# XinShuo-ph/gaussian_splatting_with_eye_tracking

Measured on AMD Instinct MI355X. Metric: rendered views/sec (fwd+bwd) at 1080p, 1M Gaussians; achieved HBM GB/s %, higher is better.
Workload: dtype fp32; 1 GPU

## Files before the change

gaussian_splatting_with_eye_tracking_amd/csrc/gs_api.cpp:

```cpp
#include <hip/hip_runtime.h>

#include <atomic>
#include <cstdio>
#include <cstdlib>
#include <chrono>
#include <cstring>
#include <functional>
#include <algorithm>
#include <deque>
#include <mutex>
#include <stdexcept>
#include <string>
#include <unordered_set>
#include <utility>
#include <vector>

#include "../../include/gsplat_amd.h"
#include "gs_kernels.h"
#include "gs_layout.h"

using namespace gsamd;

namespace {

thread_local std::string g_err;


struct GsError : std::runtime_error {
    using std::runtime_error::runtime_error;
};

#define GS_HIP_NOTHROW(expr) (void)(expr)
#define GS_HIP(expr)                                                                                  \
    do {                                                                                              \
        hipError_t _e = (expr);                                                                       \
        if (_e != hipSuccess)                                                                         \
            throw GsError(std::string(#expr) + " failed: " + hipGetErrorString(_e) + " at " __FILE__ \
                          ":" + std::to_string(__LINE__));                                            \
    } while (0)

constexpr int kStages = 15;
const char* kStageNames[kStages] = {"preprocess", "tile_scan",    "duplicate",   "sort_tiles",
                                    "render",     "render_bwd",   "bwd_gauss",   "amr_levels",
                                    "amr_render", "amr_interp",   "knn",         "zero_accum",
                                    "count_tiles", "multiview_bwd", "amr_lists"};
enum Stage {
    kPre, kScan, kDup, kSort, kRender, kRenderBwd, kBwdGauss, kAmrLevels, kAmrRender, kAmrInterp, kKnn, kZero, kCount,
    kMultiView, kAmrLists
};
struct Profiler {
    bool on = false;
    uint32_t mask = ~0u;
    struct Pending { int stage; hipEvent_t a, b; };
    std::vector<Pending> pending;
    double total_ms[kStages] = {0};
    long count[kStages] = {0};
    std::vector<hipEvent_t> pool;
    hipEvent_t get() {
        if (!pool.empty()) { hipEvent_t e = pool.back(); pool.pop_back(); return e; }
        hipEvent_t e; GS_HIP_NOTHROW(hipEventCreate(&e)); return e;
    }
    void harvest() {
        for (auto& p : pending) {
            float ms = 0.f;
            if (hipEventSynchronize(p.b) == hipSuccess && hipEventElapsedTime(&ms, p.a, p.b) == hipSuccess) {
                total_ms[p.stage] += ms; count[p.stage] += 1;
            }
            pool.push_back(p.a); pool.push_back(p.b);
        }
        pending.clear();
    }
};
Profiler g_prof;
std::mutex g_prof_mu;

thread_local DispatchEvents t_dispatch;

struct StageTimer {
    int stage; hipStream_t s; hipEvent_t a = nullptr, b = nullptr; bool on_dispatch;
    StageTimer(int st, hipStream_t str, bool dispatch = false) : stage(st), s(str), on_dispatch(dispatch) {
        if (!g_prof.on || !((g_prof.mask >> st) & 1u)) return;
        std::lock_guard<std::mutex> l(g_prof_mu);
        a = g_prof.get(); b = g_prof.get();
        if (on_dispatch) t_dispatch = DispatchEvents{a, b};
        else hipEventRecord(a, s);
    }
    ~StageTimer() {
        if (!a) return;
        if (on_dispatch) {
            const bool taken = t_dispatch.start == nullptr;
            t_dispatch = DispatchEvents{};
            std::lock_guard<std::mutex> l(g_prof_mu);
            if (taken) {
                g_prof.pending.push_back({stage, a, b});
            } else {
                g_prof.pool.push_back(a);
                g_prof.pool.push_back(b);
            }
            return;
        }
        hipEventRecord(b, s);
        std::lock_guard<std::mutex> l(g_prof_mu);
        g_prof.pending.push_back({stage, a, b});
    }
};

void stage_check(bool debug, hipStream_t s, const char* stage) {
    hipError_t e = hipGetLastError();
    if (e == hipSuccess && debug) e = hipStreamSynchronize(s);
    if (e != hipSuccess) throw GsError(std::string("[HIP ERROR] in stage ") + stage + ": " + hipGetErrorString(e));
}

uint32_t* pinned_words() {
    thread_local uint32_t* p = nullptr;
    if (!p) {
        void* q = nullptr;
        GS_HIP(hipHostMalloc(&q, 64, hipHostMallocDefault));
        p = static_cast<uint32_t*>(q);
    }
    return p;
}

int g_hdr_mirror = -1;

bool hdr_mirror_on() {
    if (g_hdr_mirror < 0) {
        const char* e = std::getenv("GSAMD_HDR_MIRROR");
        g_hdr_mirror = (e && std::atoi(e) == 0) ? 0 : 2;
    }
    return g_hdr_mirror != 0;
}
// ... 203 lines not shown
    in.store_cov3d = t_store_cov3d != 0;
    in.fwd_zero = t_fwd_zero != 0 && grad;
    in.step0_unfilled = amr && t_amr_step0_unfilled != 0;
    if (amr) t_amr_step0_unfilled = 0;
    return in;
}

PreprocessArgs make_pp(const ForwardIn& in, int tile) {
    PreprocessArgs a;
    a.P = in.P;
    a.D = in.D;
    a.M = in.M;
    a.means3D = in.means3D;
    a.scales = in.scales;
    a.scale_modifier = in.scale_modifier;
    a.rotations = in.rotations;
    a.opacities = in.opacities;
    a.shs = in.shs;
    a.cov3D_precomp = in.cov3D_precomp;
    a.colors_precomp = in.colors_precomp;
    a.viewmatrix = in.viewmatrix;
    a.projmatrix = in.projmatrix;
    a.cam_pos = in.cam_pos;
    a.W = in.width;
    a.H = in.height;
    a.tan_fovx = in.tan_fovx;
    a.tan_fovy = in.tan_fovy;
    a.focal_y = (float)in.height / (2.0f * in.tan_fovy);
    a.focal_x = (float)in.width / (2.0f * in.tan_fovx);
    a.block = tile;
    a.prefiltered = in.prefiltered;
    a.store_cov3d = in.store_cov3d;
    a.store_drgb = in.store_drgb;
    a.zero_words = nullptr;
    a.zero_n = 0;
    a.err_token = 0;
    a.antialiasing = in.antialiasing;
    return a;
}

struct Binned {
    GeomView g;
    ImageView img;
    BinningView b;
    AmrBinningView ab;
    int K;
    int T;
    int* radii;
};

int tile_count(int W, int H, int tile) { return ((W + tile - 1) / tile) * ((H + tile - 1) / tile); }

ImageView image_view(char* image, int W, int H, int tile) {
    ImageView v;
    carve_image(image, (size_t)W * H, tile_count(W, H, tile), &v, tile);
    return v;
}

Binned carve_buffers(char* geom, char* binning, char* image, int P, int K, int W, int H, int tile,
                     bool amr = false) {
    Binned r{};
    r.K = K;
    r.T = tile_count(W, H, tile);
    carve_geom(geom, P, &r.g);
    r.img = image_view(image, W, H, tile);
    carve_binning(binning, K, &r.b, amr ? &r.ab : nullptr);
    r.radii = r.g.radii;
    return r;
}

int rendered_count(int hint, char* geom, int P, const char* binning, hipStream_t s, const char* missing) {
    int K = hint;
    if (K < 0) {
        GeomView g;
        carve_geom(geom, P, &g);
        uint32_t hdr[4];
        read_header(g.hdr, hdr, s);
        K = (int)hdr[kHdrNumRendered];
    }
    if (K > 0 && !binning) throw GsError(missing);
    return K;
}

Binned preprocess_and_bin(const ForwardIn& in, const gs_buffer& geometry, const gs_buffer& binning,
                          const gs_buffer& image, int* radii, int tile, bool debug, hipStream_t s,
                          const std::function<void(Binned&)>& before_k = nullptr, int fused_sort_max = 0) {
    Binned r;
    const int W = in.width, H = in.height;
    const int gx = (W + tile - 1) / tile, gy = (H + tile - 1) / tile;
    r.T = gx * gy;
    const size_t N = (size_t)W * H;
    const bool tail = in.store_cov3d || (in.colors_precomp == nullptr && in.store_drgb);
    char* gbase = call_resize(geometry, carve_geom(nullptr, in.P, nullptr, tail, tile == 32), "geometry");
    carve_geom(gbase, in.P, &r.g);
    set_accum_clean(r.g.grad_accum, false);
    char* ibase = call_resize(image, carve_image(nullptr, N, r.T, nullptr, tile), "image");
    carve_image(ibase, N, r.T, &r.img, tile);
    r.radii = radii ? radii : r.g.radii;
    const bool lds_bin = r.T <= kLdsTiles;
    if (r.T == 0) GS_HIP(hipMemsetAsync(r.g.hdr, 0, kHdrWords * sizeof(uint32_t), s));
    if (r.T > 0 && !lds_bin) GS_HIP(hipMemsetAsync(r.img.tile_count, 0, sizeof(uint32_t) * kBinSlots * r.T, s));
    PreprocessArgs pa = make_pp(in, tile);
    pa.err_token = next_error_token();
    set_drgb_written(r.g.drgb, pa.store_drgb && in.colors_precomp == nullptr);
    if (r.T > 0 && lds_bin) {
        pa.zero_words = r.img.tile_count;
        pa.zero_n = kBinSlots * r.T;
    }
    { StageTimer _t(kPre, s); launch_preprocess(pa, r.g, r.radii, lds_bin ? nullptr : r.img.tile_count, s); }
    stage_check(debug, s, "preprocess");
    if (lds_bin) { StageTimer _t(kCount, s); launch_count_tiles(in.P, r.g, r.radii, W, H, tile, r.img, s); }
    stage_check(debug, s, "count_tiles");
    const std::pair<uint32_t*, uint32_t*> mirror =
        (r.T > 0 && hdr_mirror_on()) ? mirror_words() : std::pair<uint32_t*, uint32_t*>{nullptr, nullptr};
    const bool amr = tile == 32;
    bool dup_done = false;
    const SpecKey skey = spec_key(W, H, in.P);
    const size_t cap = (!amr && !before_k && r.T > 0 && !debug) ? spec_capacity(skey) : 0;
    const uint32_t mtoken = mirror.second ? next_mirror_token() : 0u;
    const bool pub_dup = cap > 0 && mirror.second != nullptr;
    if (r.T > 0) { StageTimer _t(kScan, s); launch_tile_scan(r.T, r.img, r.g.hdr, s, pub_dup ? nullptr : mirror.second, bin_slots_for(in.P, gx, gy, tile), gx, dup_banded(gx, gy, tile), pub_dup ? 0u : mtoken); }
    stage_check(debug, s, "tile_scan");
    uint32_t hdr[4];
    if (before_k) {
        begin_header_read(r.g.hdr, s, mirror.first);
        before_k(r);
        finish_header_read(hdr, mirror.first, s, r.g.hdr);
    } else if (cap > 0) {
        begin_header_read(r.g.hdr, s, mirror.first);
        char* sbase = call_resize(binning, carve_binning(nullptr, cap, nullptr), "binning");
        carve_binning(sbase, cap, &r.b);
        { StageTimer _t(kDup, s); launch_duplicate(in.P, r.g, r.radii, W, H, tile, r.img, r.b, s, (uint32_t)cap, r.g.hdr, (uint32_t)cap, pub_dup ? mirror.second : nullptr, pub_dup ? mtoken : 0u); }
        finish_header_read(hdr, mirror.first, s, r.g.hdr);
        dup_done = hdr[kHdrNumRendered] <= cap;
    } else if (mirror.first) {
        begin_header_read(r.g.hdr, s, mirror.first);
        finish_header_read(hdr, mirror.first, s, r.g.hdr);
    } else {
        read_header(r.g.hdr, hdr, s);
    }
    if (in.prefiltered && hdr[kHdrError] == pa.err_token)
        throw GsError("Point is filtered although prefiltered is set. This shouldn't happen!");
    r.K = (int)hdr[kHdrNumRendered];
    if (!amr) note_k(skey, r.K);
    if (!dup_done) {
        char* bbase = call_resize(binning, carve_binning(nullptr, r.K, nullptr, nullptr, amr), "binning");
        carve_binning(bbase, r.K, &r.b, amr ? &r.ab : nullptr);
    }
    if (r.K > 0) {
        if (!dup_done) { StageTimer _t(kDup, s); launch_duplicate(in.P, r.g, r.radii, W, H, tile, r.img, r.b, s, (uint32_t)r.K); }
        stage_check(debug, s, "duplicate");
        { StageTimer _t(kSort, s); launch_sort_tiles(r.T, r.img, r.b, (int)hdr[kHdrMaxTileCount], (int)hdr[kHdrNumLargeTiles], s, fused_sort_max); }
        stage_check(debug, s, "sort_tiles");
    }
    return r;
}

}

DispatchEvents gsamd::take_dispatch_events() {
    const DispatchEvents e = t_dispatch;
    t_dispatch = DispatchEvents{};
    return e;
}

extern "C" {

int gs_abi_version(void) { return GSPLAT_AMD_ABI_VERSION; }

#ifndef GSAMD_DIGEST
#define GSAMD_DIGEST "unstamped"
#endif
const char* gs_build_digest(void) { return GSAMD_DIGEST; }

const char* gs_last_error(void) { return g_err.c_str(); }

namespace {
int base_forward_impl(const ForwardIn& in, const gs_buffer& geometry, const gs_buffer& binning,
                      const gs_buffer& image, float* out_color, int* radii, bool aux, float* out_depth,
                      float* out_alpha, int debug, void* stream, const char* who) {
    const int P = in.P, width = in.width, height = in.height;
    if (aux && (!out_depth || !out_alpha)) throw GsError(std::string(who) + ": out_depth / out_alpha is NULL");
    hipStream_t s = static_cast<hipStream_t>(stream);
    if (P <= 0) {
        if (aux) {
            const size_t N = (width > 0 && height > 0) ? (size_t)width * (size_t)height : 0;
            if (N) {
                GS_HIP(hipMemsetAsync(out_depth, 0, sizeof(float) * N, s));
                GS_HIP(hipMemsetAsync(out_alpha, 0, sizeof(float) * N, s));
            }
        }
        return 0;
    }
    Binned r = preprocess_and_bin(in, geometry, binning, image, radii, 16, debug != 0, s);
    const float* feats = in.colors_precomp ? in.colors_precomp : r.g.rgb;
    bool zeroed;
    {
        StageTimer _t(kRender, s, true);
        const bool zero = in.fwd_zero;
        zeroed = launch_render_forward(width, height, r.img, r.b, r.g, feats, in.background, out_color, s,
                                       zero ? r.g.grad_accum : nullptr, zero ? (size_t)kGradRow * (size_t)P : 0,
                                       reinterpret_cast<uint8_t*>(r.b.scratch));
    }
    if (zeroed) set_accum_clean(r.g.grad_accum, true);
    stage_check(debug != 0, s, "render");
    if (aux) {
        launch_render_forward_aux(width, height, r.img, r.b, r.g, out_depth, out_alpha, s);
        stage_check(debug != 0, s, "render_aux");
    }
    return r.K;
}
}

int gs_rasterizer_forward(gs_buffer geometry, gs_buffer binning, gs_buffer image, int P, int D, int M,
                          const float* background, int width, int height, const float* means3D, const float* shs,
                          const float* colors_precomp, const float* opacities, const float* scales,
                          float scale_modifier, const float* rotations, const float* cov3D_precomp,
                          const float* viewmatrix, const float* projmatrix, const float* cam_pos, float tan_fovx,
                          float tan_fovy, int prefiltered, float* out_color, int* radii, int debug, void* stream) {
    const ForwardIn in = forward_in(false, P, D, M, background, width, height, means3D, shs, colors_precomp, opacities,
                                    scales, scale_modifier, rotations, cov3D_precomp, viewmatrix, projmatrix, cam_pos,
                                    tan_fovx, tan_fovy, prefiltered);
    return guarded([&]() -> int {
        return base_forward_impl(in, geometry, binning, image, out_color, radii, false, nullptr, nullptr, debug,
                                 stream, "gs_rasterizer_forward");
    });
}

int gs_rasterizer_forward_aux(gs_buffer geometry, gs_buffer binning, gs_buffer image, int P, int D, int M,
                              const float* background, int width, int height, const float* means3D, const float* shs,
                              const float* colors_precomp, const float* opacities, const float* scales,
                              float scale_modifier, const float* rotations, const float* cov3D_precomp,
                              const float* viewmatrix, const float* projmatrix, const float* cam_pos, float tan_fovx,
                              float tan_fovy, int prefiltered, float* out_color, int* radii, float* out_depth,
                              float* out_alpha, int debug, void* stream) {
    const ForwardIn in = forward_in(false, P, D, M, background, width, height, means3D, shs, colors_precomp, opacities,
                                    scales, scale_modifier, rotations, cov3D_precomp, viewmatrix, projmatrix, cam_pos,
                                    tan_fovx, tan_fovy, prefiltered);
    return guarded([&]() -> int {
        return base_forward_impl(in, geometry, binning, image, out_color, radii, true, out_depth, out_alpha, debug,
                                 stream, "gs_rasterizer_forward_aux");
    });
}

int gs_rasterizer_forward_ex(gs_buffer geometry, gs_buffer binning, gs_buffer image, int P, int D, int M,
                             const float* background, int width, int height, const float* means3D, const float* shs,
                             const float* colors_precomp, const float* opacities, const float* scales,
                             float scale_modifier, const float* rotations, const float* cov3D_precomp,
                             const float* viewmatrix, const float* projmatrix, const float* cam_pos, float tan_fovx,
                             float tan_fovy, int prefiltered, int antialiasing, float* out_color, int* radii,
                             float* out_depth, float* out_alpha, int debug, void* stream) {
    ForwardIn in = forward_in(false, P, D, M, background, width, height, means3D, shs, colors_precomp, opacities,
                              scales, scale_modifier, rotations, cov3D_precomp, viewmatrix, projmatrix, cam_pos,
                              tan_fovx, tan_fovy, prefiltered);
    in.antialiasing = antialiasing != 0;
    return guarded([&]() -> int {
        if ((out_depth == nullptr) != (out_alpha == nullptr))
            throw GsError("gs_rasterizer_forward_ex: out_depth and out_alpha go together (both, or both NULL)");
        return base_forward_impl(in, geometry, binning, image, out_color, radii, out_depth != nullptr, out_depth,
                                 out_alpha, debug, stream, "gs_rasterizer_forward_ex");
    });
}

namespace {
size_t det_scratch_bytes(int R) { return R > 0 ? align_up(sizeof(float) * kDetRow * (size_t)R) : 0; }

struct DetScratch {
    bool on = false;
    char* base = nullptr;
    size_t bytes = 0;
};

void check_det_scratch(const DetScratch& d, int R, const char* who) {
    if (!d.on || R <= 0) return;
    if (!d.base) throw GsError(std::string(who) + ": scratch is NULL (gs_backward_deterministic_scratch_bytes)");
    if (d.bytes < det_scratch_bytes(R))
        throw GsError(std::string(who) + ": scratch of " + std::to_string(d.bytes) + " bytes, " +
                      std::to_string(det_scratch_bytes(R)) + " needed (gs_backward_deterministic_scratch_bytes)");
// ... 756 lines not shown
        stage_check(false, s, "adam");
        return 0;
    });
}

int gs_sparse_adam_step(float* params, const float* grads, float* exp_avg, float* exp_avg_sq, long long n, int nseg,
                        const long long* seg_end, const double* lr, const long long* step, int P, const int* radii,
                        double beta1, double beta2, double eps, void* stream) {
    return guarded([&]() -> int {
        if (nseg < 1 || nseg > 8) throw GsError("gs_sparse_adam_step: 1..8 segments");
        for (int i = 0; i < nseg; i++)
            if (step[i] < 0 || (i > 0 && seg_end[i] < seg_end[i - 1]))
                throw GsError("gs_sparse_adam_step: bad segments");
        if (P < 0 || n < 0 || seg_end[0] < 0 || seg_end[nseg - 1] > n)
            throw GsError("gs_sparse_adam_step: bad sizes");
        if (P == 0 || n == 0) return 0;
        for (int i = 0; i < nseg; i++)
            if ((seg_end[i] - (i > 0 ? seg_end[i - 1] : 0)) % P != 0)
                throw GsError("gs_sparse_adam_step: every segment must hold P whole rows");
        if (!radii) throw GsError("gs_sparse_adam_step: radii is null");
        hipStream_t s = static_cast<hipStream_t>(stream);
        launch_sparse_adam(params, grads, exp_avg, exp_avg_sq, nseg, seg_end, lr, step, P, radii, beta1, beta2, eps, s);
        stage_check(false, s, "sparse_adam");
        return 0;
    });
}

long long gs_sparse_adam_rows_per_pass(void) { return sparse_adam_rows_per_pass(); }

int gs_densify_stats(int P, const int* radii, const float* grad_means2D, int grad_stride, float* xyz_gradient_accum,
                     float* denom, float* max_radii2D, void* stream) {
    return guarded([&]() -> int {
        if (P < 0 || grad_stride < 2) throw GsError("gs_densify_stats: bad sizes");
        hipStream_t s = static_cast<hipStream_t>(stream);
        launch_densify_stats(P, radii, grad_means2D, grad_stride, xyz_gradient_accum, denom, max_radii2D, s);
        stage_check(false, s, "densify_stats");
        return 0;
    });
}

int gs_activate_gaussians(int P, int M, const float* features_dc, const float* features_rest, const float* opacity_raw,
                          const float* scaling_raw, const float* rotation_raw, float* shs, float* opacities,
                          float* scales, float* rotations, void* stream) {
    return guarded([&]() -> int {
        if (P < 0 || M < 1 || M > 16) throw GsError("gs_activate_gaussians: bad sizes");
        hipStream_t s = static_cast<hipStream_t>(stream);
        launch_activate(P, M, features_dc, features_rest, opacity_raw, scaling_raw, rotation_raw, shs, opacities,
                        scales, rotations, s);
        stage_check(false, s, "activate");
        return 0;
    });
}

int gs_activation_backward(int P, int M, int accumulate, const float* dL_dshs, const float* dL_dopacities,
                           const float* dL_dscales, const float* dL_drotations, const float* dL_dmeans3D,
                           const float* opacity_raw, const float* scaling_raw, const float* rotation_raw,
                           float* grad_xyz, float* grad_features_dc, float* grad_features_rest, float* grad_opacity,
                           float* grad_scaling, float* grad_rotation, void* stream) {
    return guarded([&]() -> int {
        if (P < 0 || M < 1 || M > 16) throw GsError("gs_activation_backward: bad sizes");
        hipStream_t s = static_cast<hipStream_t>(stream);
        launch_activation_backward(P, M, accumulate, dL_dshs, dL_dopacities, dL_dscales, dL_drotations, dL_dmeans3D,
                                   opacity_raw, scaling_raw, rotation_raw, grad_xyz, grad_features_dc,
                                   grad_features_rest, grad_opacity, grad_scaling, grad_rotation, s);
        stage_check(false, s, "activation_backward");
        return 0;
    });
}

namespace {
struct TuningKey {
    const char* key;
    const int* value;
    void (*set)(int);
};
const TuningKey kTuning[] = {
    {"fwd_variant", &g_fwd_variant, set_forward_variant},
    {"bwd_variant", &g_bwd_variant, set_backward_variant},
    {"amr_variant", &g_amr_variant, set_amr_variant},
    {"sort_algo", &g_sort_algo, set_sort_algo},
    {"cull", &g_cull, set_cull},
    {"hdr_mirror", &g_hdr_mirror, [](int v) { g_hdr_mirror = v == 0 ? 0 : 2; }},
    {"spec_dup", &g_spec_dup, [](int v) { g_spec_dup = v; }},
    {"ritnet_mfma", &g_ritnet_mfma, set_ritnet_mfma},
};

const TuningKey* tuning_key(const char* key) {
    for (const TuningKey& e : kTuning)
        if (key && std::strcmp(key, e.key) == 0) return &e;
    if (key) g_err = std::string("unknown tuning key ") + key;
    return nullptr;
}
}

int gs_set_tuning(const char* key, int value) {
    const TuningKey* e = tuning_key(key);
    if (e) e->set(value);
    return e ? 0 : -1;
}

int gs_get_tuning(const char* key, int* value) {
    if (!key || !value) return -1;
    hdr_mirror_on();
    const TuningKey* e = tuning_key(key);
    if (!e) return -1;
    *value = *e->value;
    return 0;
}

int gs_set_thread_option(const char* key, int value) {
    if (!key) return -1;
    const struct { const char* key; int* value; } table[] = {{"fwd_no_grad", &t_fwd_no_grad},
                                                             {"sh_drgb", &t_sh_drgb},
                                                             {"store_cov3d", &t_store_cov3d},
                                                             {"fwd_zero", &t_fwd_zero},
                                                             {"amr_step0_unfilled", &t_amr_step0_unfilled}};
    for (const auto& e : table)
        if (std::strcmp(key, e.key) == 0) {
            *e.value = value;
            return 0;
        }
    g_err = std::string("unknown thread option ") + key;
    return -1;
}

void gs_profile_enable(int on) {
    std::lock_guard<std::mutex> l(g_prof_mu);
    g_prof.on = on != 0;
}

void gs_profile_set_mask(unsigned mask) {
    std::lock_guard<std::mutex> l(g_prof_mu);
    g_prof.mask = mask;
}

int gs_profile_stage_count(void) { return kStages; }

const char* gs_profile_stage_name(int i) { return (i >= 0 && i < kStages) ? kStageNames[i] : ""; }

void gs_profile_read(double* total_ms, long* counts, int reset) {
    std::lock_guard<std::mutex> l(g_prof_mu);
    g_prof.harvest();
    for (int i = 0; i < kStages; i++) {
        if (total_ms) total_ms[i] = g_prof.total_ms[i];
        if (counts) counts[i] = g_prof.count[i];
        if (reset) {
            g_prof.total_ms[i] = 0;
            g_prof.count[i] = 0;
        }
    }
}

size_t gs_geom_bytes(int P) { return carve_geom(nullptr, (size_t)P, nullptr); }

size_t gs_amr_geom_bytes(int P) { return carve_geom(nullptr, (size_t)P, nullptr, true, true); }

size_t gs_image_bytes(int width, int height, int tile) {
    return carve_image(nullptr, (size_t)width * height, tile_count(width, height, tile), nullptr, tile);
}

size_t gs_binning_bytes(int K) { return carve_binning(nullptr, (size_t)K, nullptr); }

namespace {
int binning_count_of_bytes(size_t nbytes, bool amr) {
    long lo = 0, hi = (long)std::min<size_t>(nbytes / 8 + 1, (size_t)INT32_MAX);
    while (lo < hi) {
// ... 51 lines not shown
```

gaussian_splatting_with_eye_tracking_amd/csrc/gs_kernels.h:

```cpp
#pragma once

#include <hip/hip_runtime.h>
#include <stdint.h>

#include "gs_layout.h"

namespace gsamd {

struct DispatchEvents {
    hipEvent_t start = nullptr, stop = nullptr;
};
DispatchEvents take_dispatch_events();

struct PreprocessArgs {
    int P, D, M;
    const float* means3D;
    const float* scales;
    float scale_modifier;
    const float* rotations;
    const float* opacities;
    const float* shs;
    const float* cov3D_precomp;
    const float* colors_precomp;
    const float* viewmatrix;
    const float* projmatrix;
    const float* cam_pos;
    int W, H;
    float tan_fovx, tan_fovy, focal_x, focal_y;
    int block;
    int prefiltered;
    int store_cov3d;
    int store_drgb;
    uint32_t* zero_words;
    int zero_n;
    uint32_t err_token;
    int antialiasing = 0;
};

void launch_preprocess(const PreprocessArgs& a, const GeomView& g, int* radii, uint32_t* tile_count,
                       hipStream_t s);
void launch_mark_visible(int P, const float* means3D, const float* viewmatrix, const float* projmatrix,
                         bool* present, hipStream_t s);

void launch_tile_scan(int T, const ImageView& img, uint32_t* hdr, hipStream_t s, uint32_t* hdr_mirror, int nslots,
                      int gx, bool banded, uint32_t mirror_token = 0);
void launch_duplicate(int P, const GeomView& g, const int* radii, int W, int H, int block, const ImageView& img,
                      const BinningView& b, hipStream_t s, uint32_t n_keys, const uint32_t* spec_hdr = nullptr,
                      uint32_t spec_cap = 0, uint32_t* mirror = nullptr, uint32_t mirror_token = 0);
constexpr int kLdsTiles = 16384;
void launch_count_tiles(int P, const GeomView& g, const int* radii, int W, int H, int block, const ImageView& img,
                        hipStream_t s);
void set_sort_algo(int v);
int bin_slots_for(int P, int gx, int gy, int block);
bool dup_banded(int gx, int gy, int block);
void launch_order_tiles(int T, const ImageView& img, bool use_max_contrib, hipStream_t s);
void launch_sort_tiles(int T, const ImageView& img, const BinningView& b, int max_count_host, int num_large_host,
                       hipStream_t s, int fused_max = 0);
constexpr int kAmrFusedSortMax = 2048;
constexpr int kAmrStepsAll = GSPLAT_AMD_AMR_STEPS_1_TO_4;
constexpr int kAmrStepsAllFill = GSPLAT_AMD_AMR_STEPS_1_TO_4_FILL;
constexpr int kAmrStepsAllSplit = GSPLAT_AMD_AMR_STEPS_1_TO_4_SPLIT;
constexpr int kAmrStateAfter = 100;
bool fused_sort_on();
void launch_reconstruct_keys(int T, const ImageView& img, const BinningView& b, const GeomView& g, uint64_t* keys,
                             hipStream_t s);

bool launch_render_forward(int W, int H, const ImageView& img, const BinningView& b, const GeomView& g,
                           const float* features, const float* bg, float* out_color, hipStream_t s,
                           float* zero_rows = nullptr, size_t zero_floats = 0, uint8_t* hit_codes = nullptr);
void launch_render_forward_aux(int W, int H, const ImageView& img, const BinningView& b, const GeomView& g,
                               float* out_depth, float* out_alpha, hipStream_t s);
void launch_render_backward_aux(int W, int H, const ImageView& img, const BinningView& b, const GeomView& g,
                                const float* colors, const float* bg, const float* dL_dpix, const float* dL_ddepth,
                                const float* dL_dalpha, hipStream_t s);
void launch_aux_depth_to_means(int P, const GeomView& g, const int* radii, const float* viewmatrix,
                               float* dL_dmean3D, hipStream_t s);
void set_forward_variant(int v);
void set_backward_variant(int v);
void set_amr_variant(int v);
void set_cull(int v);
void set_ritnet_mfma(int v);
void launch_render_backward(int W, int H, const ImageView& img, const BinningView& b, const GeomView& g,
                            const float* colors, const float* bg, const float* dL_dpix, hipStream_t s);
constexpr int kDetRow = 9;
void launch_render_backward_deterministic(int W, int H, int P, int R, const ImageView& img, const BinningView& b,
                                          const GeomView& g, const int* radii, const float* colors, const float* bg,
                                          const float* dL_dpix, float* partials, uint32_t err_token, hipStream_t s);

struct BackwardGaussArgs {
    int P, D, M;
    const float* means3D;
    const int* radii;
    const float* shs;
    const float* scales;
    const float* rotations;
    float scale_modifier;
    const float* cov3D;
    const float* viewmatrix;
    const float* projmatrix;
    const float* campos;
    float focal_x, focal_y, tan_fovx, tan_fovy;
    int has_cov_precomp;
    const float* drgb;
    const uint32_t* hdr;
    int drgb_known;
    int nt_out = 0;
    const float* opacities = nullptr;
    int antialiasing = 0;
    uint32_t* err_word = nullptr;
    uint32_t err_token = 0;
    float* dL_dmean2D;
    float* dL_dconic;
    float* dL_dopacity;
    float* dL_dcolor;
    float* dL_dmean3D;
    float* dL_dcov3D;
    float* dL_dsh;
    float* dL_dscale;
    float* dL_drot;
};
void launch_backward_gaussians(const BackwardGaussArgs& a, const GeomView& g, hipStream_t s);

constexpr int kViewRow = 10;
// ... 86 lines not shown
```

gaussian_splatting_with_eye_tracking_amd/csrc/preprocess.hip:

```cpp
#include <algorithm>

#include "gs_blend.cuh"
#include "gs_device.cuh"
#include "gs_kernels.h"

namespace gsamd {

template <bool kSH16>
__device__ __forceinline__ void load_sh(int deg, int M, const float* __restrict__ sh, float (&c)[16][3]) {
    const int ncoef = min((deg + 1) * (deg + 1), M);
    if (kSH16) {
        const float4* s4 = reinterpret_cast<const float4*>(sh);
        float buf[48];
#pragma unroll
        for (int i = 0; i < 12; i++) {
            const float4 v = (i * 4 < ncoef * 3) ? s4[i] : make_float4(0.f, 0.f, 0.f, 0.f);
            buf[4 * i + 0] = v.x; buf[4 * i + 1] = v.y; buf[4 * i + 2] = v.z; buf[4 * i + 3] = v.w;
        }
#pragma unroll
        for (int k = 0; k < 16; k++)
#pragma unroll
            for (int ch = 0; ch < 3; ch++) c[k][ch] = buf[3 * k + ch];
    } else {
#pragma unroll
        for (int k = 0; k < 16; k++)
#pragma unroll
            for (int ch = 0; ch < 3; ch++) c[k][ch] = (k < ncoef) ? sh[3 * k + ch] : 0.f;
    }
}

__device__ __forceinline__ float3 eval_sh_color(int deg, const float (&c)[16][3], float x, float y, float z,
                                                uint8_t& clamped_bits) {
    float res[3];
#pragma unroll
    for (int ch = 0; ch < 3; ch++) res[ch] = SH_C0 * c[0][ch];
    if (deg > 0) {
        const float k1 = SH_C1 * y, k2 = SH_C1 * z, k3 = SH_C1 * x;
#pragma unroll
        for (int ch = 0; ch < 3; ch++) res[ch] = res[ch] - k1 * c[1][ch] + k2 * c[2][ch] - k3 * c[3][ch];
        if (deg > 1) {
            const float xx = x * x, yy = y * y, zz = z * z;
            const float xy = x * y, yz = y * z, xz = x * z;
            const float k4 = SH_C2_0 * xy;
            const float k5 = SH_C2_1 * yz;
            const float k6 = SH_C2_2 * (2.0f * zz - xx - yy);
            const float k7 = SH_C2_3 * xz;
            const float k8 = SH_C2_4 * (xx - yy);
#pragma unroll
            for (int ch = 0; ch < 3; ch++)
                res[ch] = res[ch] + k4 * c[4][ch] + k5 * c[5][ch] + k6 * c[6][ch] + k7 * c[7][ch] + k8 * c[8][ch];
            if (deg > 2) {
                const float k9 = SH_C3_0 * y * (3.0f * xx - yy);
                const float k10 = SH_C3_1 * xy * z;
                const float k11 = SH_C3_2 * y * (4.0f * zz - xx - yy);
                const float k12 = SH_C3_3 * z * (2.0f * zz - 3.0f * xx - 3.0f * yy);
                const float k13 = SH_C3_4 * x * (4.0f * zz - xx - yy);
                const float k14 = SH_C3_5 * z * (xx - yy);
                const float k15 = SH_C3_6 * x * (xx - 3.0f * yy);
#pragma unroll
                for (int ch = 0; ch < 3; ch++)
                    res[ch] = res[ch] + k9 * c[9][ch] + k10 * c[10][ch] + k11 * c[11][ch] + k12 * c[12][ch] +
                              k13 * c[13][ch] + k14 * c[14][ch] + k15 * c[15][ch];
            }
        }
    }
    clamped_bits = 0;
#pragma unroll
    for (int ch = 0; ch < 3; ch++) {
        res[ch] += 0.5f;
        if (res[ch] < 0) clamped_bits |= (uint8_t)(1u << ch);
        res[ch] = fmaxf(res[ch], 0.0f);
    }
    return make_float3(res[0], res[1], res[2]);
}

constexpr int kPpThreads = 256;
constexpr int kShStride = 52;

template <bool kHasSH, bool kCovPrecomp, bool kAA, typename ShFn>
__device__ __forceinline__ void pp_gaussian(const PreprocessArgs& a, const GeomView& g, int* __restrict__ radii,
                                            uint32_t* __restrict__ tile_count, int idx, bool radii_copy, float mx,
                                            float my, float mz, const float (&sc)[3], float4 q, float (&cov3D)[6],
// ... 102 lines not shown
        const float4 co = make_float4(conic_x, conic_y, conic_z, opacity);
        row[0] = make_float4(pix_x, pix_y, r_, g_);
        row[1] = splat_coef(co);
        row[2] = make_float4(b_, conic_x, conic_y, conic_z);
        if (!stage) row[3] = make_float4(0.f, 0.f, 0.f, 0.f);
    }

    if (tile_count)
        for (uint32_t y = r.y0; y < r.y1; y++)
            for (uint32_t x = r.x0; x < r.x1; x++) atomicAdd(&tile_count[y * gx + x], 1u);
}

template <bool kHasSH, bool kSH16, bool kCovPrecomp, bool kDma, bool kNtIn = false, bool kAA = false>
__device__ __forceinline__ void pp_thread(const PreprocessArgs& a, const GeomView& g, int* __restrict__ radii,
                                          uint32_t* __restrict__ tile_count, int idx, const float* sh_row,
                                          float* stage) {
    const bool radii_copy = a.block == 32 && radii != g.radii;
    radii[idx] = 0;
    if (radii_copy) g.radii[idx] = 0;
    g.tiles_touched[idx] = 0;

    const float mx = ldg1<kNtIn>(a.means3D + 3 * idx + 0);
    const float my = ldg1<kNtIn>(a.means3D + 3 * idx + 1);
    const float mz = ldg1<kNtIn>(a.means3D + 3 * idx + 2);
    float sc[3] = {0.f, 0.f, 0.f};
    float4 q = make_float4(0.f, 0.f, 0.f, 0.f);
    float cov3D[6];
    if (kCovPrecomp) {
#pragma unroll
        for (int i = 0; i < 6; i++) cov3D[i] = a.cov3D_precomp[6 * idx + i];
    } else {
        sc[0] = ldg1<kNtIn>(a.scales + 3 * idx + 0);
        sc[1] = ldg1<kNtIn>(a.scales + 3 * idx + 1);
        sc[2] = ldg1<kNtIn>(a.scales + 3 * idx + 2);
        q = ldg4<kNtIn>(reinterpret_cast<const float4*>(a.rotations) + idx);
    }
    const float opacity = ldg1<kNtIn>(a.opacities + idx);
    const Mat4 V = load_mat4(a.viewmatrix);
    const Mat4 Pm = load_mat4(a.projmatrix);
    pp_gaussian<kHasSH, kCovPrecomp, kAA>(a, g, radii, tile_count, idx, radii_copy, mx, my, mz, sc, q, cov3D, opacity,
                                     V, Pm, [&](float (&shc)[16][3]) {
        if constexpr (kDma) {
            asm volatile("s_waitcnt vmcnt(0)" ::: "memory");
            const int ncoef = min((a.D + 1) * (a.D + 1), a.M);
            typedef float f4v __attribute__((ext_vector_type(4)));
            float v[48];
#pragma unroll
            for (int i = 0; i < 12; i++) {
                f4v t = reinterpret_cast<const f4v*>(sh_row)[i];
                asm volatile("" : "+v"(t));
                v[4 * i] = t.x; v[4 * i + 1] = t.y; v[4 * i + 2] = t.z; v[4 * i + 3] = t.w;
            }
#pragma unroll
            for (int k = 0; k < 16; k++)
#pragma unroll
                for (int ch = 0; ch < 3; ch++) shc[k][ch] = k < ncoef ? v[3 * k + ch] : 0.f;
        } else {
            load_sh<kSH16>(a.D, a.M, a.shs + (size_t)idx * a.M * 3, shc);
        }
    }, stage);
}

template <bool kHasSH, bool kSH16, bool kCovPrecomp, bool kDma = false, bool kAA = false>
__global__ void __launch_bounds__(kPpThreads) preprocess_kernel(PreprocessArgs a, GeomView g, int* __restrict__ radii,
                                                                uint32_t* __restrict__ tile_count) {
    static_assert(!kDma || (kHasSH && kSH16), "LDS-DMA stages 16-coefficient SH rows");
    constexpr bool kStageOut = kDma, kNtIn = kDma;
    const int idx = blockIdx.x * blockDim.x + threadIdx.x;
    __shared__ __attribute__((aligned(16))) float s_sh[kDma ? kPpThreads * kShStride : 1];
    if constexpr (kDma) {
        const int w = threadIdx.x >> 6, lane = threadIdx.x & 63;
        const size_t row0 = (size_t)blockIdx.x * kPpThreads + 64 * w;
        const float* src = a.shs + row0 * 48;
        float* dst = s_sh + 64 * kShStride * w;
        constexpr int kPieces = kShStride / 4;
#pragma unroll
        for (int i = 0; i < kPieces; i++) {
            const int p = 64 * i + lane, r = p / kPieces, j = p - kPieces * r;
            if (j < 12 && row0 + (size_t)r < (size_t)a.P)
                __builtin_amdgcn_global_load_lds(src + 48 * r + 4 * j, dst + 256 * i, 16, 0, 2);
        }
    }
    for (int i = idx; i < a.zero_n; i += (int)(gridDim.x * blockDim.x)) a.zero_words[i] = 0u;
    if (idx == 0) g.hdr[kHdrDrgb] = (kHasSH && a.store_drgb) ? 1u : 0u;
    if (idx == 0) g.hdr[kHdrAntialias] = kAA ? 1u : 0u;
    float* row = s_sh + (kDma ? kShStride * threadIdx.x : 0);
    if constexpr (kStageOut) {
        const int wrow0 = (int)(blockIdx.x * kPpThreads) + (int)(threadIdx.x & ~63u);
        if (wrow0 >= a.P) return;
        if (idx < a.P) pp_thread<kHasSH, kSH16, kCovPrecomp, kDma, kNtIn, kAA>(a, g, radii, tile_count, idx, row, row);
        __builtin_amdgcn_fence(__ATOMIC_RELEASE, "wavefront");
        __builtin_amdgcn_wave_barrier();
        __builtin_amdgcn_fence(__ATOMIC_ACQUIRE, "wavefront");
        const int lane = threadIdx.x & 63;
        const float* wl = s_sh + kShStride * (threadIdx.x & ~63u);
        const int nrow = min(64, a.P - wrow0);
        if (a.store_drgb) {
            float4* out = reinterpret_cast<float4*>(g.drgb) + 3 * (size_t)wrow0;
#pragma unroll
            for (int i = 0; i < 3; i++) {
                const int c = lane + 64 * i;
                if (c < 3 * nrow) {
                    const float4 v = *reinterpret_cast<const float4*>(wl + kShStride * (c / 3) + 4 * (c % 3));
                    typedef float f4v __attribute__((ext_vector_type(4)));
                    __builtin_nontemporal_store(f4v{v.x, v.y, v.z, v.w}, reinterpret_cast<f4v*>(out + c));
                }
            }
        }
        if (a.block == 32) {
            float4* out = reinterpret_cast<float4*>(g.amr_rows + (size_t)16 * wrow0);
#pragma unroll
            for (int i = 0; i < 4; i++) {
                const int c = lane + 64 * i;
                if (c < 4 * nrow)
                    out[c] = (c & 3) == 3 ? make_float4(0.f, 0.f, 0.f, 0.f)
                                          : *reinterpret_cast<const float4*>(wl + kShStride * (c >> 2) + 16 + 4 * (c & 3));
            }
        }
        const int nf = 3 * nrow;
        if (4 * lane < nf) {
            float v4[4];
#pragma unroll
            for (int e = 0; e < 4; e++) {
                const int f = min(4 * lane + e, nf - 1);
                v4[e] = wl[kShStride * (f / 3) + 12 + f % 3];
            }
            float* out = g.rgb + 3 * (size_t)wrow0 + 4 * lane;
            if (4 * lane + 4 <= nf) {
                *reinterpret_cast<float4*>(out) = make_float4(v4[0], v4[1], v4[2], v4[3]);
            } else {
#pragma unroll
                for (int e = 0; e < 3; e++)
                    if (4 * lane + e < nf) out[e] = v4[e];
            }
        }
        return;
    }
    if (idx >= a.P) return;
    pp_thread<kHasSH, kSH16, kCovPrecomp, kDma, false, kAA>(a, g, radii, tile_count, idx, row, nullptr);
}

template <bool A, bool B, bool C>
static void launch_pp(const PreprocessArgs& a, const GeomView& g, int* radii, uint32_t* tile_count, hipStream_t s) {
    const int blocks = (a.P + kPpThreads - 1) / kPpThreads;
    if (a.antialiasing && a.block == 16)
        hipLaunchKernelGGL((preprocess_kernel<A, B, C, A && B, true>), dim3(blocks), dim3(kPpThreads), 0, s, a, g,
                           radii, tile_count);
    else
        hipLaunchKernelGGL((preprocess_kernel<A, B, C, A && B>), dim3(blocks), dim3(kPpThreads), 0, s, a, g, radii,
                           tile_count);
}

void launch_preprocess(const PreprocessArgs& a, const GeomView& g, int* radii, uint32_t* tile_count,
                       hipStream_t s) {
    if (a.P == 0) return;
    const bool has_sh = a.colors_precomp == nullptr;
    const bool sh16 = has_sh && a.M == 16;
    const bool covp = a.cov3D_precomp != nullptr;
    if (has_sh) {
        if (sh16) {
            if (covp) launch_pp<true, true, true>(a, g, radii, tile_count, s);
            else launch_pp<true, true, false>(a, g, radii, tile_count, s);
        } else {
            if (covp) launch_pp<true, false, true>(a, g, radii, tile_count, s);
            else launch_pp<true, false, false>(a, g, radii, tile_count, s);
        }
    } else {
        if (covp) launch_pp<false, false, true>(a, g, radii, tile_count, s);
        else launch_pp<false, false, false>(a, g, radii, tile_count, s);
    }
}

__global__ void __launch_bounds__(256) mark_visible_kernel(int P, const float* __restrict__ means3D,
                                                           const float* __restrict__ viewmatrix,
                                                           bool* __restrict__ present) {
    const int idx = blockIdx.x * blockDim.x + threadIdx.x;
    if (idx >= P) return;
    const Mat4 V = load_mat4(viewmatrix);
    const float3 pv = transform_point_4x3(means3D[3 * idx], means3D[3 * idx + 1], means3D[3 * idx + 2], V);
    present[idx] = !(pv.z <= 0.2f);
}

void launch_mark_visible(int P, const float* means3D, const float* viewmatrix, const float* projmatrix,
                         bool* present, hipStream_t s) {
    (void)projmatrix;
    if (P == 0) return;
    hipLaunchKernelGGL(mark_visible_kernel, dim3((P + 255) / 256), dim3(256), 0, s, P, means3D, viewmatrix,
                       present);
}

}
```

Baseline: 1274 views/s.

## Fork SH colour evaluation onto a side stream overlapping binning in forward

```diff
diff --git a/gaussian_splatting_with_eye_tracking_amd/csrc/gs_api.cpp b/gaussian_splatting_with_eye_tracking_amd/csrc/gs_api.cpp
--- a/gaussian_splatting_with_eye_tracking_amd/csrc/gs_api.cpp
+++ b/gaussian_splatting_with_eye_tracking_amd/csrc/gs_api.cpp
@@ -39,14 +39,14 @@
                           ":" + std::to_string(__LINE__));                                            \
     } while (0)
 
-constexpr int kStages = 15;
+constexpr int kStages = 16;
 const char* kStageNames[kStages] = {"preprocess", "tile_scan",    "duplicate",   "sort_tiles",
                                     "render",     "render_bwd",   "bwd_gauss",   "amr_levels",
                                     "amr_render", "amr_interp",   "knn",         "zero_accum",
-                                    "count_tiles", "multiview_bwd", "amr_lists"};
+                                    "count_tiles", "multiview_bwd", "amr_lists",  "sh_colour"};
 enum Stage {
     kPre, kScan, kDup, kSort, kRender, kRenderBwd, kBwdGauss, kAmrLevels, kAmrRender, kAmrInterp, kKnn, kZero, kCount,
-    kMultiView, kAmrLists
+    kMultiView, kAmrLists, kShColour
 };
 struct Profiler {
     bool on = false;
@@ -416,9 +416,54 @@
     return K;
 }
 
+int g_fwd_fork = 1;
+
+struct ForkLane {
+    hipStream_t side = nullptr;
+    hipEvent_t forked = nullptr;
+    hipEvent_t joined = nullptr;
+    int cus = 0;
+};
+ForkLane& fork_lane() {
+    thread_local std::vector<ForkLane> per_device;
+    int dev = 0;
+    GS_HIP(hipGetDevice(&dev));
+    if ((int)per_device.size() <= dev) per_device.resize(dev + 1);
+    ForkLane& l = per_device[dev];
+    if (!l.forked) GS_HIP(hipEventCreateWithFlags(&l.forked, hipEventDisableTiming));
+    if (!l.joined) GS_HIP(hipEventCreateWithFlags(&l.joined, hipEventDisableTiming));
+    if (!l.side) GS_HIP(hipStreamCreateWithFlags(&l.side, hipStreamNonBlocking));
+    if (!l.cus) GS_HIP(hipDeviceGetAttribute(&l.cus, hipDeviceAttributeMultiprocessorCount, dev));
+    return l;
+}
+int colour_blocks(const ForkLane& l, int P) {
+    const int nchunks = (P + 255) / 256;
+    return std::max(l.cus, (nchunks + 15) / 16);
+}
+
+struct ForkJoin {
+    hipStream_t s = nullptr, side = nullptr;
+    hipEvent_t joined = nullptr;
+    bool armed = false, recorded = false;
+    ForkJoin() = default;
+    ForkJoin(const ForkJoin&) = delete;
+    ForkJoin& operator=(const ForkJoin&) = delete;
+    hipError_t wait() {
+        armed = false;
+        if (!recorded) {
+            const hipError_t e = hipEventRecord(joined, side);
+            if (e != hipSuccess) return e;
+        }
+        return hipStreamWaitEvent(s, joined, 0);
+    }
+    void join() { if (armed) GS_HIP(wait()); }
+    ~ForkJoin() { if (armed) GS_HIP_NOTHROW(wait()); }
+};
+
 Binned preprocess_and_bin(const ForwardIn& in, const gs_buffer& geometry, const gs_buffer& binning,
                           const gs_buffer& image, int* radii, int tile, bool debug, hipStream_t s,
-                          const std::function<void(Binned&)>& before_k = nullptr, int fused_sort_max = 0) {
+                          const std::function<void(Binned&)>& before_k = nullptr, int fused_sort_max = 0,
+                          ForkJoin* fork = nullptr) {
     Binned r;
     const int W = in.width, H = in.height;
     const int gx = (W + tile - 1) / tile, gy = (H + tile - 1) / tile;
@@ -441,7 +486,20 @@
         pa.zero_words = r.img.tile_count;
         pa.zero_n = kBinSlots * r.T;
     }
-    { StageTimer _t(kPre, s); launch_preprocess(pa, r.g, r.radii, lds_bin ? nullptr : r.img.tile_count, s); }
+    const bool forked = fork && g_fwd_fork != 0 && tile == 16 && in.colors_precomp == nullptr && !debug && r.T > 0;
+    pa.split_colour = forked ? 1 : 0;
+    if (!forked) {
+        StageTimer _t(kPre, s);
+        launch_preprocess(pa, r.g, r.radii, lds_bin ? nullptr : r.img.tile_count, s);
+    } else {
+        ForkLane& lane = fork_lane();
+        { StageTimer _t(kPre, s); launch_preprocess(pa, r.g, r.radii, lds_bin ? nullptr : r.img.tile_count, s, lane.forked); }
+        GS_HIP(hipStreamWaitEvent(lane.side, lane.forked, 0));
+        fork->s = s; fork->side = lane.side; fork->joined = lane.joined;
+        fork->armed = true;
+        { StageTimer _t(kShColour, lane.side); launch_sh_colour(pa, r.g, r.radii, lane.side, colour_blocks(lane, in.P), lane.joined); }
+        fork->recorded = true;
+    }
     stage_check(debug, s, "preprocess");
     if (lds_bin) { StageTimer _t(kCount, s); launch_count_tiles(in.P, r.g, r.radii, W, H, tile, r.img, s); }
     stage_check(debug, s, "count_tiles");
@@ -526,8 +584,10 @@
         }
         return 0;
     }
-    Binned r = preprocess_and_bin(in, geometry, binning, image, radii, 16, debug != 0, s);
+    ForkJoin fork;
+    Binned r = preprocess_and_bin(in, geometry, binning, image, radii, 16, debug != 0, s, nullptr, 0, &fork);
     const float* feats = in.colors_precomp ? in.colors_precomp : r.g.rgb;
+    fork.join();
     bool zeroed;
     {
         StageTimer _t(kRender, s, true);
@@ -1450,6 +1510,7 @@
     {"cull", &g_cull, set_cull},
     {"hdr_mirror", &g_hdr_mirror, [](int v) { g_hdr_mirror = v == 0 ? 0 : 2; }},
     {"spec_dup", &g_spec_dup, [](int v) { g_spec_dup = v; }},
+    {"fwd_fork", &g_fwd_fork, [](int v) { g_fwd_fork = v != 0; }},
     {"ritnet_mfma", &g_ritnet_mfma, set_ritnet_mfma},
 };
 
diff --git a/gaussian_splatting_with_eye_tracking_amd/csrc/gs_kernels.h b/gaussian_splatting_with_eye_tracking_amd/csrc/gs_kernels.h
--- a/gaussian_splatting_with_eye_tracking_amd/csrc/gs_kernels.h
+++ b/gaussian_splatting_with_eye_tracking_amd/csrc/gs_kernels.h
@@ -35,10 +35,13 @@
     int zero_n;
     uint32_t err_token;
     int antialiasing = 0;
+    int split_colour = 0;
 };
 
 void launch_preprocess(const PreprocessArgs& a, const GeomView& g, int* radii, uint32_t* tile_count,
-                       hipStream_t s);
+                       hipStream_t s, hipEvent_t done = nullptr);
+void launch_sh_colour(const PreprocessArgs& a, const GeomView& g, const int* radii, hipStream_t s,
+                      int max_blocks = 0, hipEvent_t done = nullptr);
 void launch_mark_visible(int P, const float* means3D, const float* viewmatrix, const float* projmatrix,
                          bool* present, hipStream_t s);
 
diff --git a/gaussian_splatting_with_eye_tracking_amd/csrc/preprocess.hip b/gaussian_splatting_with_eye_tracking_amd/csrc/preprocess.hip
--- a/gaussian_splatting_with_eye_tracking_amd/csrc/preprocess.hip
+++ b/gaussian_splatting_with_eye_tracking_amd/csrc/preprocess.hip
@@ -1,3 +1,5 @@
+#include <hip/hip_ext.h>
+
 #include <algorithm>
 
 #include "gs_blend.cuh"
@@ -266,7 +268,7 @@
         }
     }
     for (int i = idx; i < a.zero_n; i += (int)(gridDim.x * blockDim.x)) a.zero_words[i] = 0u;
-    if (idx == 0) g.hdr[kHdrDrgb] = (kHasSH && a.store_drgb) ? 1u : 0u;
+    if (idx == 0) g.hdr[kHdrDrgb] = ((kHasSH || a.split_colour) && a.store_drgb) ? 1u : 0u;
     if (idx == 0) g.hdr[kHdrAntialias] = kAA ? 1u : 0u;
     float* row = s_sh + (kDma ? kShStride * threadIdx.x : 0);
     if constexpr (kStageOut) {
@@ -325,8 +327,18 @@
 }
 
 template <bool A, bool B, bool C>
-static void launch_pp(const PreprocessArgs& a, const GeomView& g, int* radii, uint32_t* tile_count, hipStream_t s) {
+static void launch_pp(const PreprocessArgs& a, const GeomView& g, int* radii, uint32_t* tile_count, hipStream_t s,
+                      hipEvent_t done) {
     const int blocks = (a.P + kPpThreads - 1) / kPpThreads;
+    if (done) {
+        if (a.antialiasing && a.block == 16)
+            hipExtLaunchKernelGGL((preprocess_kernel<A, B, C, A && B, true>), dim3(blocks), dim3(kPpThreads), 0, s,
+                                  nullptr, done, 0, a, g, radii, tile_count);
+        else
+            hipExtLaunchKernelGGL((preprocess_kernel<A, B, C, A && B>), dim3(blocks), dim3(kPpThreads), 0, s, nullptr,
+                                  done, 0, a, g, radii, tile_count);
+        return;
+    }
     if (a.antialiasing && a.block == 16)
         hipLaunchKernelGGL((preprocess_kernel<A, B, C, A && B, true>), dim3(blocks), dim3(kPpThreads), 0, s, a, g,
                            radii, tile_count);
@@ -336,23 +348,161 @@
 }
 
 void launch_preprocess(const PreprocessArgs& a, const GeomView& g, int* radii, uint32_t* tile_count,
-                       hipStream_t s) {
+                       hipStream_t s, hipEvent_t done) {
     if (a.P == 0) return;
-    const bool has_sh = a.colors_precomp == nullptr;
+    const bool has_sh = a.colors_precomp == nullptr && !a.split_colour;
     const bool sh16 = has_sh && a.M == 16;
     const bool covp = a.cov3D_precomp != nullptr;
     if (has_sh) {
         if (sh16) {
-            if (covp) launch_pp<true, true, true>(a, g, radii, tile_count, s);
-            else launch_pp<true, true, false>(a, g, radii, tile_count, s);
+            if (covp) launch_pp<true, true, true>(a, g, radii, tile_count, s, done);
+            else launch_pp<true, true, false>(a, g, radii, tile_count, s, done);
         } else {
-            if (covp) launch_pp<true, false, true>(a, g, radii, tile_count, s);
-            else launch_pp<true, false, false>(a, g, radii, tile_count, s);
+            if (covp) launch_pp<true, false, true>(a, g, radii, tile_count, s, done);
+            else launch_pp<true, false, false>(a, g, radii, tile_count, s, done);
         }
     } else {
-        if (covp) launch_pp<false, false, true>(a, g, radii, tile_count, s);
-        else launch_pp<false, false, false>(a, g, radii, tile_count, s);
-    }
+        if (covp) launch_pp<false, false, true>(a, g, radii, tile_count, s, done);
+        else launch_pp<false, false, false>(a, g, radii, tile_count, s, done);
+    }
+}
+
+__device__ __forceinline__ void sh_rows_dma(const PreprocessArgs& a, float* s_sh, int chunk) {
+    const int w = threadIdx.x >> 6, lane = threadIdx.x & 63;
+    const size_t row0 = (size_t)chunk * kPpThreads + 64 * w;
+    const float* src = a.shs + row0 * 48;
+    float* dst = s_sh + 64 * kShStride * w;
+    constexpr int kPieces = kShStride / 4;
+#pragma unroll
+    for (int i = 0; i < kPieces; i++) {
+        const int p = 64 * i + lane, r = p / kPieces, j = p - kPieces * r;
+        if (j < 12 && row0 + (size_t)r < (size_t)a.P)
+            __builtin_amdgcn_global_load_lds(src + 48 * r + 4 * j, dst + 256 * i, 16, 0, 2);
+    }
+}
+
+__device__ __forceinline__ void read_sh_row(const PreprocessArgs& a, const float* sh_row, float (&shc)[16][3]) {
+    asm volatile("s_waitcnt vmcnt(0)" ::: "memory");
+    const int ncoef = min((a.D + 1) * (a.D + 1), a.M);
+    typedef float f4v __attribute__((ext_vector_type(4)));
+    float v[48];
+#pragma unroll
+    for (int i = 0; i < 12; i++) {
+        f4v t = reinterpret_cast<const f4v*>(sh_row)[i];
+        asm volatile("" : "+v"(t));
+        v[4 * i] = t.x; v[4 * i + 1] = t.y; v[4 * i + 2] = t.z; v[4 * i + 3] = t.w;
+    }
+#pragma unroll
+    for (int k = 0; k < 16; k++)
+#pragma unroll
+        for (int ch = 0; ch < 3; ch++) shc[k][ch] = k < ncoef ? v[3 * k + ch] : 0.f;
+}
+
+__device__ __forceinline__ void store_wave_drgb(const GeomView& g, const float* wl, int wrow0, int nrow, int lane) {
+    float4* out = reinterpret_cast<float4*>(g.drgb) + 3 * (size_t)wrow0;
+#pragma unroll
+    for (int i = 0; i < 3; i++) {
+        const int c = lane + 64 * i;
+        if (c < 3 * nrow) {
+            const float4 v = *reinterpret_cast<const float4*>(wl + kShStride * (c / 3) + 4 * (c % 3));
+            typedef float f4v __attribute__((ext_vector_type(4)));
+            __builtin_nontemporal_store(f4v{v.x, v.y, v.z, v.w}, reinterpret_cast<f4v*>(out + c));
+        }
+    }
+}
+
+__device__ __forceinline__ void store_wave_rgb(const GeomView& g, const float* wl, int wrow0, int nrow, int lane) {
+    const int nf = 3 * nrow;
+    if (4 * lane < nf) {
+        float v4[4];
+#pragma unroll
+        for (int e = 0; e < 4; e++) {
+            const int f = min(4 * lane + e, nf - 1);
+            v4[e] = wl[kShStride * (f / 3) + 12 + f % 3];
+        }
+        float* out = g.rgb + 3 * (size_t)wrow0 + 4 * lane;
+        if (4 * lane + 4 <= nf) {
+            *reinterpret_cast<float4*>(out) = make_float4(v4[0], v4[1], v4[2], v4[3]);
+        } else {
+#pragma unroll
+            for (int e = 0; e < 3; e++)
+                if (4 * lane + e < nf) out[e] = v4[e];
+        }
+    }
+}
+
+template <bool kSH16>
+__device__ __forceinline__ void colour_thread(const PreprocessArgs& a, const GeomView& g, int idx, float mx, float my,
+                                              float mz, const float* sh_row, float* stage) {
+    float shc[16][3];
+    if constexpr (kSH16) read_sh_row(a, sh_row, shc);
+    else load_sh<false>(a.D, a.M, a.shs + (size_t)idx * a.M * 3, shc);
+    float dx = mx - a.cam_pos[0], dy = my - a.cam_pos[1], dz = mz - a.cam_pos[2];
+    const float len = sqrtf(dot3(dx, dy, dz, dx, dy, dz));
+    dx = dx / len; dy = dy / len; dz = dz / len;
+    uint8_t cbits;
+    const float3 rgb = eval_sh_color(a.D, shc, dx, dy, dz, cbits);
+    if (a.store_drgb) {
+        float dx3[3], dy3[3], dz3[3];
+        sh_ddir(a.D, shc, dx, dy, dz, dx3, dy3, dz3);
+        float4* row = stage ? reinterpret_cast<float4*>(stage)
+                            : reinterpret_cast<float4*>(g.drgb) + 3 * (size_t)idx;
+        row[0] = make_float4(dx3[0], dx3[1], dx3[2], dy3[0]);
+        row[1] = make_float4(dy3[1], dy3[2], dz3[0], dz3[1]);
+        row[2] = make_float4(dz3[2], 0.f, 0.f, 0.f);
+    }
+    if (stage) {
+        *reinterpret_cast<float4*>(stage + 12) = make_float4(rgb.x, rgb.y, rgb.z, 0.f);
+    } else {
+        g.rgb[3 * idx + 0] = rgb.x;
+        g.rgb[3 * idx + 1] = rgb.y;
+        g.rgb[3 * idx + 2] = rgb.z;
+    }
+    g.clamped[idx] = cbits;
+}
+
+template <bool kSH16>
+__global__ void __launch_bounds__(kPpThreads) sh_colour_kernel(PreprocessArgs a, GeomView g,
+                                                               const int* __restrict__ radii, int nchunks) {
+    __shared__ __attribute__((aligned(16))) float s_sh[kSH16 ? kPpThreads * kShStride : 1];
+    for (int chunk = blockIdx.x; chunk < nchunks; chunk += gridDim.x) {
+        const int idx = chunk * kPpThreads + threadIdx.x;
+        const int ci = min(idx, a.P - 1);
+        const int radius = radii[ci];
+        const float mx = a.means3D[3 * ci + 0], my = a.means3D[3 * ci + 1], mz = a.means3D[3 * ci + 2];
+        if constexpr (kSH16) {
+            sh_rows_dma(a, s_sh, chunk);
+            float* row = s_sh + kShStride * threadIdx.x;
+            const int wrow0 = chunk * kPpThreads + (int)(threadIdx.x & ~63u);
+            if (wrow0 >= a.P) return;
+            if (idx < a.P && radius > 0) colour_thread<true>(a, g, idx, mx, my, mz, row, row);
+            __builtin_amdgcn_fence(__ATOMIC_RELEASE, "wavefront");
+            __builtin_amdgcn_wave_barrier();
+            __builtin_amdgcn_fence(__ATOMIC_ACQUIRE, "wavefront");
+            const int lane = threadIdx.x & 63;
+            const float* wl = s_sh + kShStride * (threadIdx.x & ~63u);
+            const int nrow = min(64, a.P - wrow0);
+            if (a.store_drgb) store_wave_drgb(g, wl, wrow0, nrow, lane);
+            store_wave_rgb(g, wl, wrow0, nrow, lane);
+            asm volatile("s_waitcnt vmcnt(0) lgkmcnt(0)" ::: "memory");
+            __builtin_amdgcn_wave_barrier();
+        } else {
+            if (idx < a.P && radius > 0) colour_thread<false>(a, g, idx, mx, my, mz, nullptr, nullptr);
+        }
+    }
+}
+
+void launch_sh_colour(const PreprocessArgs& a, const GeomView& g, const int* radii, hipStream_t s, int max_blocks,
+                      hipEvent_t done) {
+    if (a.P == 0) return;
+    const int nchunks = (a.P + kPpThreads - 1) / kPpThreads;
+    const int blocks = max_blocks > 0 ? std::min(nchunks, max_blocks) : nchunks;
+    if (a.M == 16)
+        hipExtLaunchKernelGGL(sh_colour_kernel<true>, dim3(blocks), dim3(kPpThreads), 0, s, nullptr, done, 0, a, g,
+                              radii, nchunks);
+    else
+        hipExtLaunchKernelGGL(sh_colour_kernel<false>, dim3(blocks), dim3(kPpThreads), 0, s, nullptr, done, 0, a, g,
+                              radii, nchunks);
 }
 
 __global__ void __launch_bounds__(256) mark_visible_kernel(int P, const float* __restrict__ means3D,
```

After: 1302 views/s, median of 6. +2.2%, better.
